# westlake-repl/Adapter4Rec

Measured on NVIDIA B200. Metric: train user-sequences/s (SASRec + BERT-base LoRA r=8 adapter-tuning step: fwd+bwd+allreduce+Adam), higher is better.
Workload: dtype bf16

## Files before the change

adapter4rec_b200/csrc/attention_small.cu:

```cuda
#include "a4r_common.cuh"
#include "mma_sync.cuh"

namespace {

constexpr int LP = 32;
constexpr int WARPS_PER_CTA = 4;

struct AttnParams {
  const __nv_bfloat16* qkv;
  __nv_bfloat16* out;
  const __nv_bfloat16* dout;
  const void* mask;
  int64_t ld_qkv, ld_out, mask_ld;
  int N, L, heads;
  int mask_dtype;
  const int32_t* cu_seqlens;
  int causal;
  float scale, mask_neg;
  uint32_t drop_thr16;
  float drop_scale;
  uint64_t drop_seed, drop_offset;
};

A4R_DEVICE void prob_dropout(float (&s)[2][4][4], const AttnParams& p, int n, int h, int lane) {
// ... 237 lines not shown
      uint32_t a0[4], a1[4];
      acc_to_a(a0, s[0][2 * ks], s[0][2 * ks + 1]);
      acc_to_a(a1, s[1][2 * ks], s[1][2 * ks + 1]);
#pragma unroll
      for (int np = 0; np < DH / 16; ++np) {
        uint32_t b[4];
        load_b_kn<DH>(b, sV, np * 16, ks * 16, lane);
        const uint32_t b0[2] = {b[0], b[1]}, b1[2] = {b[2], b[3]};
        mma_bf16_16816(o[0][np * 2], a0, b0);
        mma_bf16_16816(o[0][np * 2 + 1], a0, b1);
        mma_bf16_16816(o[1][np * 2], a1, b0);
        mma_bf16_16816(o[1][np * 2 + 1], a1, b1);
      }
    }
    __syncwarp();
    acc_to_tile<DH, DH / 8>(my, o, 1.f, 1.f, 1.f, 1.f, lane);
    __syncwarp();
    store_tile<DH>(my, p.out + sq.row0 * p.ld_out + h * DH, p.ld_out, sq.L, lane);
    __syncwarp();
  }
}

template <int DH>
__global__ void __launch_bounds__(WARPS_PER_CTA * 32) attn_bwd_kernel(const AttnParams p) {
  extern __shared__ __align__(128) uint8_t smem_attn[];
  constexpr int TB = Tile<DH>::kBytes;
  constexpr int PB = Tile<32>::kBytes;
  const int warp = threadIdx.x >> 5, lane = threadIdx.x & 31;
  uint8_t* my = smem_attn + warp * (4 * TB + 2 * PB);
  const int64_t total = static_cast<int64_t>(p.N) * p.heads;
  for (int64_t w = static_cast<int64_t>(blockIdx.x) * WARPS_PER_CTA + warp; w < total;
       w += static_cast<int64_t>(gridDim.x) * WARPS_PER_CTA) {
    const int n = static_cast<int>(w / p.heads), h = static_cast<int>(w % p.heads);
    const int64_t Hd = static_cast<int64_t>(p.heads) * DH;
    const SeqSpan sq = seq_span(p, n);
    const __nv_bfloat16* q = p.qkv + sq.row0 * p.ld_qkv + h * DH;
    uint8_t *tQ = my, *tK = my + TB, *tV = my + 2 * TB, *tdO = my + 3 * TB, *tP = my + 4 * TB, *tdS = tP + PB;
    load_tile<DH>(tQ, q, p.ld_qkv, sq.L, lane);
    load_tile<DH>(tK, q + Hd, p.ld_qkv, sq.L, lane);
    load_tile<DH>(tV, q + 2 * Hd, p.ld_qkv, sq.L, lane);
    load_tile<DH>(tdO, p.dout + sq.row0 * p.ld_out + h * DH, p.ld_out, sq.L, lane);
    const uint32_t km = build_keymask(p, sq, lane);
    cp_async_wait_all();
    __syncwarp();
    const uint32_t sQ = smem_u32(tQ), sK = smem_u32(tK), sV = smem_u32(tV), sdO = smem_u32(tdO), sP = smem_u32(tP),
                   sdS = smem_u32(tdS);
    float s[2][4][4];
    scores_softmax<DH>(s, sQ, sK, p, sq.L, lane, km);
    float dp[2][4][4];
#pragma unroll
    for (int mt = 0; mt < 2; ++mt)
#pragma unroll
      for (int nt = 0; nt < 4; ++nt)
#pragma unroll
        for (int e = 0; e < 4; ++e) dp[mt][nt][e] = 0.0f;
#pragma unroll
// ... 94 lines not shown
        mma_bf16_16816(dk[0][np * 2 + 1], a0, b1);
        mma_bf16_16816(dk[1][np * 2], a1, b0);
        mma_bf16_16816(dk[1][np * 2 + 1], a1, b1);
        uint32_t c[4];
        load_b_kn<DH>(c, sdO, np * 16, ks * 16, lane);
        const uint32_t c0[2] = {c[0], c[1]}, c1[2] = {c[2], c[3]};
        mma_bf16_16816(dv[0][np * 2], p0, c0);
        mma_bf16_16816(dv[0][np * 2 + 1], p0, c1);
        mma_bf16_16816(dv[1][np * 2], p1, c0);
        mma_bf16_16816(dv[1][np * 2 + 1], p1, c1);
      }
    }
    __syncwarp();
    acc_to_tile<DH, DH / 8>(tQ, acc, 1.f, 1.f, 1.f, 1.f, lane);
    acc_to_tile<DH, DH / 8>(tK, dk, 1.f, 1.f, 1.f, 1.f, lane);
    acc_to_tile<DH, DH / 8>(tV, dv, 1.f, 1.f, 1.f, 1.f, lane);
    __syncwarp();
    __nv_bfloat16* dq = p.out + sq.row0 * p.ld_qkv + h * DH;
    store_tile<DH>(tQ, dq, p.ld_qkv, sq.L, lane);
    store_tile<DH>(tK, dq + Hd, p.ld_qkv, sq.L, lane);
    store_tile<DH>(tV, dq + 2 * Hd, p.ld_qkv, sq.L, lane);
    __syncwarp();
  }
}

int check_common(const a4r_attn_args* a) {
  A4R_CHECK_ARG(a != nullptr, "attention: args is NULL");
  A4R_CHECK_ARG(a->qkv && a->out, "attention: qkv/out must be non-NULL");
  A4R_CHECK_ARG(a->L >= 1 && a->L <= LP, "attention_small: L must be in [1,32] (got %lld)", (long long)a->L);
  A4R_CHECK_ARG(a->head_dim == 32 || a->head_dim == 64, "attention_small: head_dim must be 32 or 64");
  A4R_CHECK_ARG(a->heads >= 1 && a->N >= 0, "attention: bad heads/N");
  A4R_CHECK_ARG(a->ld_qkv >= 3 * a->heads * a->head_dim && a->ld_qkv % 8 == 0, "attention: bad ld_qkv");
  A4R_CHECK_ARG(a->ld_out >= a->heads * a->head_dim && a->ld_out % 8 == 0, "attention: bad ld_out");
  A4R_CHECK_ARG(a4r_aligned16(a->qkv) && a4r_aligned16(a->out), "attention: pointers must be 16B aligned");
  A4R_CHECK_ARG(a->mask_dtype >= 0 && a->mask_dtype <= 2, "attention: mask_dtype must be 0,1,2");
  if (a->mask_dtype != 0)
    A4R_CHECK_ARG(a->mask != nullptr && (a->cu_seqlens != nullptr || a->mask_ld >= a->L), "attention: bad mask/mask_ld");
  A4R_CHECK_ARG(a->dropout_p >= 0.0f && a->dropout_p < 1.0f, "attention: dropout_p must be in [0,1)");
  return a4r_device_check();
}

AttnParams to_params(const a4r_attn_args* a) {
  AttnParams p;
  p.qkv = static_cast<const __nv_bfloat16*>(a->qkv);
  p.out = static_cast<__nv_bfloat16*>(a->out);
  p.dout = static_cast<const __nv_bfloat16*>(a->dout);
// ... 38 lines not shown
  int rc = check_common(a);
  if (rc != A4R_OK) return rc;
  if (a->N == 0) return A4R_OK;
  const AttnParams p = to_params(a);
  static bool done64 = false, done32 = false;
  if (a->head_dim == 64)
    return launch(attn_fwd_kernel<64>, WARPS_PER_CTA * 3 * Tile<64>::kBytes, p, static_cast<cudaStream_t>(stream), &done64);
  return launch(attn_fwd_kernel<32>, WARPS_PER_CTA * 3 * Tile<32>::kBytes, p, static_cast<cudaStream_t>(stream), &done32);
}

extern "C" int a4r_attn_small_bwd(const a4r_attn_args* a, a4r_stream_t stream) {
  int rc = check_common(a);
  if (rc != A4R_OK) return rc;
  A4R_CHECK_ARG(a->dout != nullptr && a4r_aligned16(a->dout), "attention bwd: dout missing or unaligned");
  if (a->N == 0) return A4R_OK;
  const AttnParams p = to_params(a);
  static bool done64 = false, done32 = false;
  if (a->head_dim == 64)
    return launch(attn_bwd_kernel<64>, WARPS_PER_CTA * (4 * Tile<64>::kBytes + 2 * Tile<32>::kBytes), p,
                  static_cast<cudaStream_t>(stream), &done64);
  return launch(attn_bwd_kernel<32>, WARPS_PER_CTA * (4 * Tile<32>::kBytes + 2 * Tile<32>::kBytes), p,
                static_cast<cudaStream_t>(stream), &done32);
}
```

adapter4rec_b200/functional.py:

```python
import torch

from . import ops

BF16 = torch.bfloat16


PARAM_EPOCH = [0]


def bump_param_epoch():
    PARAM_EPOCH[0] += 1


class WeightCache:

    def __init__(self):
        self.key = None
        self.master = None
        self.w = None
        self.wt = None

    def get(self, weight, need_t=False):
        key = (weight.data_ptr(), weight._version, weight.device, PARAM_EPOCH[0] if weight.requires_grad else -1)
        if key != self.key:
# ... 256 lines not shown


def dropout_add(x, res, p):
    return DropoutAddFunction.apply(x, res, float(p))


class AddFunction(torch.autograd.Function):

    @staticmethod
    def forward(ctx, x, res):
        return ops.dropout(x.contiguous(), res.contiguous(), 0.0, 0, 0)

    @staticmethod
    def backward(ctx, dy):
        return (dy if ctx.needs_input_grad[0] else None), (dy if ctx.needs_input_grad[1] else None)


def add(x, res):
    return AddFunction.apply(x, res)


class AttentionFunction(torch.autograd.Function):
    @staticmethod
    def forward(ctx, qkv, mask, N, L, heads, head_dim, causal, mask_neg, dropout_p=0.0, scale=None, cu_seqlens=None):
        ctx.cfg = (N, L, heads, head_dim, causal, mask_neg, scale)
        ctx.cu = cu_seqlens
        ctx.mask = mask
        ctx.drop = None
        if dropout_p > 0.0:
            ctx.drop = (dropout_p,) + DropoutState.draw(N * heads * 32 * 8)
        out, lse = ops.attn_small_fwd(qkv, N, L, heads, head_dim, mask=mask, causal=causal, mask_neg=mask_neg, want_lse=True,
                                      dropout=ctx.drop, scale=scale, cu_seqlens=cu_seqlens)
        ctx.save_for_backward(qkv, lse, out if lse is not None else None)
        return out

    @staticmethod
    def backward(ctx, dctx):
        qkv, lse, out = ctx.saved_tensors
        N, L, heads, head_dim, causal, mask_neg, scale = ctx.cfg
        dqkv = ops.attn_small_bwd(qkv, dctx.contiguous(), N, L, heads, head_dim, mask=ctx.mask, causal=causal,
                                  mask_neg=mask_neg, lse=lse, ctx=out, dropout=ctx.drop, scale=scale, cu_seqlens=ctx.cu)
        return dqkv, None, None, None, None, None, None, None, None, None, None


def attention(qkv, mask, N, L, heads, head_dim, causal=False, mask_neg=ops.F32_MIN, dropout_p=0.0, scale=None,
              cu_seqlens=None):
    return AttentionFunction.apply(qkv, mask, N, L, heads, head_dim, causal, mask_neg, float(dropout_p), scale, cu_seqlens)


class GatherRowsFunction(torch.autograd.Function):

    @staticmethod
    def forward(ctx, x, idx):
        ctx.rows = x.shape[0]
        ctx.save_for_backward(idx)
        return ops.gather_rows(x.contiguous(), idx)

    @staticmethod
    def backward(ctx, dy):
        (idx,) = ctx.saved_tensors
        dx = torch.zeros((ctx.rows, dy.shape[1]), dtype=dy.dtype, device=dy.device)
        dx.index_copy_(0, idx, dy.contiguous())
        return dx, None


def gather_rows(x, idx):
    return GatherRowsFunction.apply(x, idx)


class ExpandRowsFunction(torch.autograd.Function):
# ... 94 lines not shown
                for j, o, r in slots:
                    st[0][o:o + r].copy_(params[4 * j + 2].detach())
                    torch.mul(params[4 * j + 3].detach(), 1.0 / r, out=st[1][j * H:(j + 1) * H, o:o + r])
                a_cat, a_cat_t = ops.cast_transpose(st[0], True, True)
                b_ext, b_ext_t = ops.cast_transpose(st[1], True, True)
                tb = cache.get("t_bias_const")
                if tb is None or tb[0] != ctx.ones_col or tb[1].device != dev:
                    t_bias = torch.zeros(LORA_PAD, dtype=torch.float32, device=dev)
                    if ctx.ones_col:
                        t_bias[LORA_PAD - 1] = 1.0
                    tb = cache["t_bias_const"] = (ctx.ones_col, t_bias)
                t_bias = tb[1]
                cache["a_cat"], cache["b_ext"], cache["t_bias"] = a_cat, b_ext, t_bias
                cache["a_cat_t"], cache["b_ext_t"] = a_cat_t, b_ext_t
            T = ops.gemm(x, a_cat, bias=t_bias)
            qkv = ops.gemm(x, w, bias=bias, a2=T, b2=b_ext)
        else:
            qkv = ops.gemm(x, w, bias=bias)
        ctx.cache, ctx.slots, ctx.H, ctx.n = cache, slots, H, n
        if not slots:
            ctx.ones_col = False
        ctx.n_params = len(params)
        ctx.param_needs = [p is not None and p.requires_grad for p in params]
        need_x = any(ctx.param_needs[4 * j + 2] for j in range(n)) or any(ctx.param_needs[4 * j] for j in range(n))
        ctx.save_for_backward(x if need_x else None, T, a_cat, b_ext)
        if ctx.with_skip:
            return qkv, x
        return qkv

    @staticmethod
    def backward(ctx, dqkv, dskip=None):
        x, T, a_cat, b_ext = ctx.saved_tensors
        H, cache, n = ctx.H, ctx.cache, ctx.n
        tail = (None,) if ctx.with_skip else ()
        if dqkv is None:
            return (dskip, None) + (None,) * ctx.n_params + tail
        dqkv = dqkv.contiguous()
        if dskip is not None:
            dskip = dskip.contiguous()
        if cache.get("wt") is None:
            cache["wt"] = cache["w"].t().contiguous()
        grads = [None] * ctx.n_params
        dT = None
        if ctx.slots:
            if cache.get("b_ext") is b_ext and cache.get("b_ext_t") is not None:
                b_ext_t, a_cat_t = cache["b_ext_t"], cache["a_cat_t"]
            else:
                b_ext_t, a_cat_t = b_ext.t().contiguous(), a_cat.t().contiguous()
                if cache.get("b_ext") is b_ext:
                    cache["b_ext_t"], cache["a_cat_t"] = b_ext_t, a_cat_t
            lj = [j for j, _, _ in ctx.slots]
            if n == 3 and len(lj) == 2:
                (ja, jb) = lj
                dT = ops.gemm(dqkv[:, ja * H:(ja + 1) * H], b_ext_t[:, ja * H:(ja + 1) * H],
                              a2=dqkv[:, jb * H:(jb + 1) * H], b2=b_ext_t[:, jb * H:(jb + 1) * H])
            elif n == 3 and len(lj) == 1:
                dT = ops.gemm(dqkv[:, lj[0] * H:(lj[0] + 1) * H], b_ext_t[:, lj[0] * H:(lj[0] + 1) * H])
            else:
                dT = ops.gemm(dqkv, b_ext_t)
            dx = ops.gemm(dqkv, cache["wt"], a2=dT, b2=a_cat_t, residual=dskip) if ctx.needs_input_grad[0] else None
        else:
            dx = ops.gemm(dqkv, cache["wt"], residual=dskip) if ctx.needs_input_grad[0] else None
        fused = bool(ctx.slots) and ctx.ones_col
        if fused:
            want_g1 = any(ctx.param_needs[4 * j + 1] for j in range(n)) or any(ctx.param_needs[4 * j + 3] for j, _, _ in ctx.slots)
            want_g2 = any(ctx.param_needs[4 * j + 2] for j, _, _ in ctx.slots)
            g1_rows = [ctx.param_needs[4 * j + 1] or any(jj == j and ctx.param_needs[4 * j + 3] for jj, _, _ in ctx.slots)
                       for j in range(n)]
            g1 = [None] * n
            if want_g1:
                if all(g1_rows):
                    full = ops.wgrad(dqkv, T)
                    g1 = [full[j * H:(j + 1) * H] for j in range(n)]
                else:
                    g1 = [ops.wgrad(dqkv[:, j * H:(j + 1) * H], T) if g1_rows[j] else None for j in range(n)]
            g2 = ops.wgrad(dT, x) if want_g2 else None
        for j in range(n):
            dq = dqkv[:, j * H:(j + 1) * H]
            if ctx.param_needs[4 * j]:
                grads[4 * j] = ops.wgrad(dq, x)
            if ctx.param_needs[4 * j + 1]:
                grads[4 * j + 1] = g1[j][:, LORA_PAD - 1].contiguous() if fused else ops.colsum(dq)
        for j, o, r in ctx.slots:
            dq = dqkv[:, j * H:(j + 1) * H]
            if ctx.param_needs[4 * j + 3]:
                grads[4 * j + 3] = (g1[j][:, o:o + r] * (1.0 / r)) if fused else \
                    _pad_cols_wgrad(dq, T, o, r, 1.0 / r, transpose=False)
            if ctx.param_needs[4 * j + 2]:
                grads[4 * j + 2] = g2[o:o + r].contiguous() if fused else _pad_cols_wgrad(dT, x, o, r, 1.0, transpose=True)
        return (dx, None) + tuple(grads) + tail


def _pad_cols_wgrad(a, b, off, r, alpha, transpose):
    lo = (off // 8) * 8
    hi = ((off + r + 7) // 8) * 8
    if transpose:
        full = ops.wgrad(a[:, lo:hi], b, alpha=alpha)
        return full[off - lo:off - lo + r].contiguous()
    full = ops.wgrad(a, b[:, lo:hi], alpha=alpha)
    return full[:, off - lo:off - lo + r].contiguous()


class EmbedLNFunction(torch.autograd.Function):

    @staticmethod
    def forward(ctx, ids, L, tables, gamma, beta, eps, roberta_pad_id, prompt, word_pad_idx, *params):
        word, pos, typ = tables
        need_prompt = prompt is not None and prompt.requires_grad
        need_tab = [p is not None and p.requires_grad for p in params] + [False] * (5 - len(params))
        need = need_prompt or any(need_tab)
# ... 254 lines not shown
```

adapter4rec_b200/lib.py:

```python
import ctypes
import os
from ctypes import POINTER, Structure, c_char_p, c_float, c_int32, c_int64, c_size_t, c_void_p

HERE = os.path.dirname(os.path.abspath(__file__))
LIB_PATH = os.path.join(HERE, "libadapter4rec_sm100.so")

A4R_OK, A4R_EINVAL, A4R_ECUDA, A4R_EARCH, A4R_EWORKSPACE = 0, -1, -2, -3, -4
EPI_LINEAR, EPI_GELU, EPI_RELU, EPI_DGELU, EPI_DRELU = 0, 1, 2, 3, 4


class GemmArgs(Structure):
    _fields_ = [
        ("A", c_void_p), ("lda", c_int64), ("B", c_void_p), ("ldb", c_int64),
        ("A2", c_void_p), ("lda2", c_int64), ("B2", c_void_p), ("ldb2", c_int64), ("K2", c_int64),
        ("C", c_void_p), ("ldc", c_int64), ("aux", c_void_p), ("ldaux", c_int64),
        ("residual", c_void_p), ("ldr", c_int64), ("residual2", c_void_p), ("ldr2", c_int64),
        ("bias", c_void_p), ("M", c_int64), ("N", c_int64), ("K", c_int64),
        ("alpha", c_float), ("epilogue", c_int32), ("out_f32", c_int32), ("block_n", c_int32),
        ("dropout_p", c_float), ("dropout_seed", ctypes.c_uint64), ("dropout_offset", ctypes.c_uint64),
        ("dropout_after_residual", c_int32),
    ]


class AttnArgs(Structure):
    _fields_ = [
        ("qkv", c_void_p), ("out", c_void_p), ("dout", c_void_p), ("mask", c_void_p),
        ("ld_qkv", c_int64), ("ld_out", c_int64), ("mask_ld", c_int64),
        ("N", c_int64), ("L", c_int64), ("heads", c_int64), ("head_dim", c_int64),
        ("mask_dtype", c_int32), ("causal", c_int32), ("scale", c_float), ("mask_neg", c_float),
        ("lse", c_void_p), ("ctx", c_void_p),
        ("dropout_p", c_float), ("dropout_seed", ctypes.c_uint64), ("dropout_offset", ctypes.c_uint64),
        ("cu_seqlens", c_void_p),
    ]


class EmbedArgs(Structure):
    _fields_ = [
        ("ids", c_void_p), ("ld_ids", c_int64), ("word_emb", c_void_p), ("pos_emb", c_void_p),
        ("type_emb", c_void_p), ("prompt", c_void_p), ("gamma", c_void_p), ("beta", c_void_p),
        ("out", c_void_p), ("z_out", c_void_p), ("mean_out", c_void_p), ("rstd_out", c_void_p),
        ("N", c_int64), ("L", c_int64), ("H", c_int64), ("pos_offset", c_int64),
        ("roberta_pad_id", c_int64), ("n_prompt", c_int64), ("eps", c_float),
    ]


class BceArgs(Structure):
    _fields_ = [
        ("prec", c_void_p), ("emb", c_void_p), ("log_mask", c_void_p), ("pos_score", c_void_p),
        ("neg_score", c_void_p), ("loss", c_void_p), ("count", c_void_p),
        ("B", c_int64), ("S", c_int64), ("D", c_int64), ("cpc", c_int32),
    ]


class AdapterArgs(Structure):
    _fields_ = [
# ... 2 lines not shown
        ("gamma", c_void_p), ("beta", c_void_p), ("out", c_void_p), ("z_out", c_void_p),
        ("mean", c_void_p), ("rstd", c_void_p), ("s_out", c_void_p), ("u_out", c_void_p),
        ("M", c_int64), ("H", c_int64), ("r", c_int64), ("act", c_int32), ("tail", c_int32), ("eps", c_float),
        ("lds", c_int64), ("impl", c_int32),
    ]


class InbatchCeArgs(Structure):
    _fields_ = [
        ("prec", c_void_p), ("cand", c_void_p), ("ld_cand", c_int64), ("item_ids", c_void_p), ("log_mask", c_void_p),
        ("cand_bias", c_void_p), ("lse", c_void_p), ("loss", c_void_p), ("count", c_void_p),
        ("B", c_int64), ("S", c_int64), ("D", c_int64), ("masked_logit", c_float),
    ]


PROTOTYPES = {
    "a4r_version": (c_int32, []),
    "a4r_last_error_string": (c_char_p, []),
    "a4r_device_check": (c_int32, []),
    "a4r_launch_count": (c_int64, []),
    "a4r_gemm_bf16_tn": (c_int32, [POINTER(GemmArgs), c_void_p]),
    "a4r_attn_small_fwd": (c_int32, [POINTER(AttnArgs), c_void_p]),
    "a4r_attn_small_bwd": (c_int32, [POINTER(AttnArgs), c_void_p]),
    "a4r_attn_mid_fwd": (c_int32, [POINTER(AttnArgs), c_void_p]),
    "a4r_attn_mid_bwd": (c_int32, [POINTER(AttnArgs), c_void_p]),
    "a4r_layernorm_fwd": (c_int32, [c_void_p, c_void_p, c_int64, c_void_p, c_void_p, c_float, c_void_p, c_void_p,
                                    c_void_p, c_void_p, c_int64, c_int64, c_void_p]),
    "a4r_layernorm_bwd_workspace_bytes": (c_size_t, [c_int64]),
    "a4r_layernorm_bwd": (c_int32, [c_void_p, c_void_p, c_void_p, c_void_p, c_void_p, c_void_p, c_void_p, c_void_p,
                                    c_int32, c_void_p, c_size_t, c_int64, c_int64, c_void_p, c_float, ctypes.c_uint64,
                                    ctypes.c_uint64, c_void_p]),
    "a4r_layernorm_bwd_add": (c_int32, [c_void_p, c_void_p, c_void_p, c_void_p, c_void_p, c_void_p, c_void_p, c_int64, c_int64,
                                        c_void_p]),
    "a4r_adapter_ln_supported": (c_int32, [c_int64, c_int64]),
    "a4r_adapter_ln_fwd": (c_int32, [POINTER(AdapterArgs), c_void_p]),
    "a4r_embed_ln_fwd": (c_int32, [POINTER(EmbedArgs), c_void_p]),
    "a4r_act_bwd": (c_int32, [c_void_p, c_void_p, c_void_p, c_int64, c_int32, c_void_p]),
    "a4r_act_fwd": (c_int32, [c_void_p, c_void_p, c_int64, c_int32, c_void_p]),
    "a4r_scatter_add_rows": (c_int32, [c_void_p, c_int64, c_void_p, c_void_p, c_int64, c_int64, c_int64, c_int64, c_void_p]),
    "a4r_cast_transpose_f32_bf16": (c_int32, [c_void_p, c_int64, c_void_p, c_void_p, c_int64, c_int64, c_void_p]),
    "a4r_dropout": (c_int32, [c_void_p, c_void_p, c_void_p, c_int64, c_float, ctypes.c_uint64, ctypes.c_uint64, c_void_p]),
    "a4r_colsum_workspace_bytes": (c_size_t, [c_int64]),
    "a4r_colsum": (c_int32, [c_void_p, c_int64, c_int64, c_int64, c_void_p, c_int32, c_void_p, c_size_t, c_void_p]),
    "a4r_wgrad_workspace_bytes": (c_size_t, [c_int64, c_int64, c_int64]),
    "a4r_wgrad_bf16": (c_int32, [c_void_p, c_int64, c_void_p, c_int64, c_void_p, c_int64, c_int64, c_int64, c_int64,
                                 c_float, c_int32, c_void_p, c_size_t, c_void_p]),
# ... 57 lines not shown
```

adapter4rec_b200/model/bert.py:

```python
import torch
import torch.nn as nn

from .. import functional as Fn
from .. import ops
from .layers import BF16, Embedding, LayerNorm, Linear, LoRALinear, to_2d_bf16


class TextConfigLite:

    def __init__(self, hf_config=None, **kw):
        src = {} if hf_config is None else {k: getattr(hf_config, k) for k in dir(hf_config) if not k.startswith("_")
                                            and isinstance(getattr(hf_config, k, None), (int, float, str, bool, type(None)))}
        src.update(kw)
        self.vocab_size = src.get("vocab_size", 30522)
        self.hidden_size = src.get("hidden_size", 768)
        self.num_hidden_layers = src.get("num_hidden_layers", 12)
        self.num_attention_heads = src.get("num_attention_heads", 12)
        self.intermediate_size = src.get("intermediate_size", 3072)
        self.max_position_embeddings = src.get("max_position_embeddings", 512)
        self.type_vocab_size = src.get("type_vocab_size", 2)
        self.layer_norm_eps = src.get("layer_norm_eps", 1e-12)
        self.pad_token_id = src.get("pad_token_id", 0)
        self.model_type = src.get("model_type", "bert")
        self.hidden_dropout_prob = src.get("hidden_dropout_prob", 0.1)
# ... 26 lines not shown
        tables = (table, self.position_embeddings.table_bf16(), typ)
        g, b = self.LayerNorm.weight.detach().float(), self.LayerNorm.bias.detach().float()
        wmaster = we.wte.weight if hasattr(we, "learned_embedding") else we.weight
        masters = [wmaster, self.position_embeddings.weight, self.token_type_embeddings.weight, self.LayerNorm.weight,
                   self.LayerNorm.bias]
        masters = [m if m.requires_grad else None for m in masters]
        x = Fn.EmbedLNFunction.apply(input_ids, L, tables, g, b, self.LayerNorm.eps, roberta_pad, prompt,
                                     int(self.config.pad_token_id), *masters)
        if self.training and self.dropout.p > 0:
            x = Fn.dropout_add(x, None, self.dropout.p)
        return x


class BertSelfAttention(nn.Module):
    def __init__(self, config):
        super().__init__()
        self.num_attention_heads = config.num_attention_heads
        self.attention_head_size = config.hidden_size // config.num_attention_heads
        self.all_head_size = config.hidden_size
        self.query = Linear(config.hidden_size, config.hidden_size)
        self.key = Linear(config.hidden_size, config.hidden_size)
        self.value = Linear(config.hidden_size, config.hidden_size)
        self.dropout = nn.Dropout(config.attention_probs_dropout_prob)
        self._qkv_cache = {}

    def forward(self, x2d, attention_mask, N, L, packed=None, want_skip=False):
        params = []
        for m in (self.query, self.key, self.value):
            params += [m.weight, m.bias, getattr(m, "lora_A", None), getattr(m, "lora_B", None)]
        skip = x2d
        if want_skip and x2d.requires_grad:
            qkv, skip = Fn.QKVFunction.apply(x2d, self._qkv_cache, *params, "skip")
        else:
            qkv = Fn.QKVFunction.apply(x2d, self._qkv_cache, *params)
        if packed is not None:
            ctx = Fn.attention(qkv, packed.token_mask, N, L, self.num_attention_heads, self.attention_head_size,
                               causal=False, mask_neg=ops.F32_MIN, dropout_p=self.dropout.p if self.training else 0.0,
                               cu_seqlens=packed.cu_seqlens)
        else:
            ctx = Fn.attention(qkv, attention_mask, N, L, self.num_attention_heads, self.attention_head_size,
                               causal=False, mask_neg=ops.F32_MIN, dropout_p=self.dropout.p if self.training else 0.0)
        return (ctx, skip) if want_skip else ctx


class BertSelfOutput(nn.Module):

    def __init__(self, config, in_features=None):
        super().__init__()
        self.dense = Linear(in_features or config.hidden_size, config.hidden_size)
        self.LayerNorm = LayerNorm(config.hidden_size, eps=config.layer_norm_eps)
        self.dropout = nn.Dropout(config.hidden_dropout_prob)

    def forward(self, hidden_states, input_tensor):
        shape = input_tensor.shape
        p = self.dropout.p if self.training else 0.0
        d = self.dense
        if not (d.weight.requires_grad or d.bias.requires_grad):
            out = Fn.PostLNBlockFunction.apply(to_2d_bf16(hidden_states), to_2d_bf16(input_tensor), self.LayerNorm.weight,
                                               self.LayerNorm.bias, self.LayerNorm.eps, p, d.weight, d.bias, d._cache,
                                               None, None, None)
            return out.view(shape)
        if p > 0:
            z = Fn.dropout_add(d(to_2d_bf16(hidden_states)), to_2d_bf16(input_tensor).contiguous(), p)
        else:
# ... 150 lines not shown
```

adapter4rec_b200/ops.py:

```python
import ctypes

import torch

from . import lib as _l
from .lib import EPI_DGELU, EPI_DRELU, EPI_GELU, EPI_LINEAR, EPI_RELU

BF16 = torch.bfloat16
F32_MIN = -3.4028234663852886e38


def _stream():
    return ctypes.c_void_p(torch.cuda.current_stream().cuda_stream)


def _p(t):
    return None if t is None else ctypes.c_void_p(t.data_ptr())


def _rows2d(t, name):
    if t.dim() != 2 or t.stride(1) != 1:
        raise ValueError("%s must be 2-D with unit column stride, got shape %s stride %s" % (name, tuple(t.shape), t.stride()))
    return t.stride(0) if t.shape[0] > 1 else max(t.stride(0), t.shape[1])


# ... 132 lines not shown
        lse = torch.empty((N * L, heads), dtype=torch.float32, device=qkv.device)
        a.lse = _p(lse)
    fn, name = _attn_kernel(L, head_dim, causal, "fwd")
    _l.check(fn(ctypes.byref(a), _stream()), name)
    return (out, lse) if want_lse else out


def attn_small_bwd(qkv, dctx, N, L, heads, head_dim, mask=None, causal=False, mask_neg=F32_MIN, lse=None, ctx=None,
                   dropout=None, scale=None, cu_seqlens=None):
    assert qkv.dtype == BF16 and dctx.dtype == BF16 and dctx.shape[0] == qkv.shape[0]
    assert cu_seqlens is not None or qkv.shape[0] == N * L
    dqkv = torch.empty((qkv.shape[0], 3 * heads * head_dim), dtype=BF16, device=qkv.device)
    a = _attn_args(qkv, N, L, heads, head_dim, mask, causal, mask_neg, dropout, scale, cu_seqlens)
    assert _rows2d(qkv, "qkv") == dqkv.stride(0), "attention bwd expects a contiguous qkv"
    a.out, a.dout, a.ld_out = _p(dqkv), _p(dctx), _rows2d(dctx, "dctx")
    if L > 32:
        assert lse is not None and ctx is not None and ctx.is_contiguous() and dctx.is_contiguous()
        a.lse, a.ctx = _p(lse), _p(ctx)
    fn, name = _attn_kernel(L, head_dim, causal, "bwd")
    _l.check(fn(ctypes.byref(a), _stream()), name)
    return dqkv


def layernorm_fwd(x, gamma, beta, eps, res=None, want_z=False, want_stats=True):
    assert x.dtype == BF16 and x.is_contiguous() and x.dim() == 2
    M, H = x.shape
    y = torch.empty_like(x)
    z = torch.empty_like(x) if want_z else None
    mean = torch.empty(M, dtype=torch.float32, device=x.device) if want_stats else None
    rstd = torch.empty(M, dtype=torch.float32, device=x.device) if want_stats else None
    res_rows = 0
    if res is not None:
        assert res.dtype == BF16 and res.is_contiguous() and res.shape[-1] == H
        res_rows = res.numel() // H
    _l.check(_l.get_lib().a4r_layernorm_fwd(_p(x), _p(res), res_rows, _p(gamma), _p(beta), float(eps), _p(y), _p(z),
                                            _p(mean), _p(rstd), M, H, _stream()), "a4r_layernorm_fwd")
    return y, z, mean, rstd


def layernorm_bwd(dy, z, mean, rstd, gamma, dgamma=None, dbeta=None, accumulate=False, masked=None):
    assert dy.dtype == BF16 and z.dtype == BF16 and dy.is_contiguous() and z.is_contiguous()
    M, H = z.shape
    dz = torch.empty_like(z)
    dzm = torch.empty_like(z) if masked is not None else None
    mp, mseed, moff = masked if masked is not None else (0.0, 0, 0)
    ws, wsb = None, 0
# ... 389 lines not shown
```

include/adapter4rec.h:

```cpp
#ifndef ADAPTER4REC_H_
#define ADAPTER4REC_H_

#include <stddef.h>
#include <stdint.h>

#ifdef __cplusplus
extern "C" {
#endif

#define A4R_OK 0
#define A4R_EINVAL (-1)
#define A4R_ECUDA (-2)
#define A4R_EARCH (-3)
#define A4R_EWORKSPACE (-4)

typedef void* a4r_stream_t;

#define A4R_API __attribute__((visibility("default")))

A4R_API int a4r_version(void);
A4R_API const char* a4r_last_error_string(void);
A4R_API int a4r_device_check(void);
A4R_API int64_t a4r_launch_count(void);

// ... 39 lines not shown

typedef struct a4r_attn_args {
  const void* qkv;
  void* out;
  const void* dout;
  const void* mask;
  int64_t ld_qkv, ld_out, mask_ld;
  int64_t N, L, heads, head_dim;
  int32_t mask_dtype;
  int32_t causal;
  float scale;
  float mask_neg;
  float* lse;
  const void* ctx;
  float dropout_p;
  uint64_t dropout_seed;
  uint64_t dropout_offset;
  const int32_t* cu_seqlens;
} a4r_attn_args;

A4R_API int a4r_attn_small_fwd(const a4r_attn_args* args, a4r_stream_t stream);
A4R_API int a4r_attn_small_bwd(const a4r_attn_args* args, a4r_stream_t stream);

A4R_API int a4r_attn_mid_fwd(const a4r_attn_args* args, a4r_stream_t stream);
A4R_API int a4r_attn_mid_bwd(const a4r_attn_args* args, a4r_stream_t stream);

A4R_API int a4r_layernorm_fwd(const void* x, const void* res, int64_t res_rows, const float* gamma, const float* beta,
                      float eps, void* y, void* z_out, float* mean, float* rstd, int64_t M, int64_t H,
                      a4r_stream_t stream);
A4R_API size_t a4r_layernorm_bwd_workspace_bytes(int64_t H);
A4R_API int a4r_layernorm_bwd(const void* dy, const void* z, const float* mean, const float* rstd, const float* gamma,
                      void* dz, float* dgamma, float* dbeta, int32_t accumulate, void* workspace,
                      size_t workspace_bytes, int64_t M, int64_t H, void* dz_masked, float dropout_p,
                      uint64_t dropout_seed, uint64_t dropout_offset, a4r_stream_t stream);
A4R_API int a4r_layernorm_bwd_add(const void* dy, const void* z, const float* mean, const float* rstd, const float* gamma,
                          const void* dskip, void* dz, int64_t M, int64_t H, a4r_stream_t stream);

typedef struct a4r_adapter_args {
  const void* h;
  int64_t ldh;
  const void* input;
  int64_t ldi;
  const void* w_down;
  const float* b_down;
  const void* w_up;
  const float* b_up;
// ... 136 lines not shown
```

Baseline: 2010.

## Fuse LoRA-B gradient and dT computation into the attention backward kernel via clusters

New measurement: 1733, median of 6. -13.8%, worse.

```diff
diff --git a/adapter4rec_b200/csrc/attention_small.cu b/adapter4rec_b200/csrc/attention_small.cu
--- a/adapter4rec_b200/csrc/attention_small.cu
+++ b/adapter4rec_b200/csrc/attention_small.cu
@@ -283,16 +283,10 @@
 }
 
 template <int DH>
-__global__ void __launch_bounds__(WARPS_PER_CTA * 32) attn_bwd_kernel(const AttnParams p) {
-  extern __shared__ __align__(128) uint8_t smem_attn[];
+A4R_DEVICE void bwd_head(const AttnParams& p, int n, int h, uint8_t* my, int lane) {
   constexpr int TB = Tile<DH>::kBytes;
   constexpr int PB = Tile<32>::kBytes;
-  const int warp = threadIdx.x >> 5, lane = threadIdx.x & 31;
-  uint8_t* my = smem_attn + warp * (4 * TB + 2 * PB);
-  const int64_t total = static_cast<int64_t>(p.N) * p.heads;
-  for (int64_t w = static_cast<int64_t>(blockIdx.x) * WARPS_PER_CTA + warp; w < total;
-       w += static_cast<int64_t>(gridDim.x) * WARPS_PER_CTA) {
-    const int n = static_cast<int>(w / p.heads), h = static_cast<int>(w % p.heads);
+  {
     const int64_t Hd = static_cast<int64_t>(p.heads) * DH;
     const SeqSpan sq = seq_span(p, n);
     const __nv_bfloat16* q = p.qkv + sq.row0 * p.ld_qkv + h * DH;
@@ -433,6 +427,194 @@
     store_tile<DH>(tV, dq + 2 * Hd, p.ld_qkv, sq.L, lane);
     __syncwarp();
   }
+}
+
+template <int DH>
+__global__ void __launch_bounds__(WARPS_PER_CTA * 32) attn_bwd_kernel(const AttnParams p) {
+  extern __shared__ __align__(128) uint8_t smem_attn[];
+  const int warp = threadIdx.x >> 5, lane = threadIdx.x & 31;
+  uint8_t* my = smem_attn + warp * (4 * Tile<DH>::kBytes + 2 * Tile<32>::kBytes);
+  const int64_t total = static_cast<int64_t>(p.N) * p.heads;
+  for (int64_t w = static_cast<int64_t>(blockIdx.x) * WARPS_PER_CTA + warp; w < total;
+       w += static_cast<int64_t>(gridDim.x) * WARPS_PER_CTA)
+    bwd_head<DH>(p, static_cast<int>(w / p.heads), static_cast<int>(w % p.heads), my, lane);
+}
+
+constexpr int LORA_W = 8;
+constexpr int LORA_G = LORA_W + 1;
+constexpr int kLoraStage = 32 * 2 * LORA_W;
+constexpr int kLoraAcc = 2 * 64 * LORA_G;
+constexpr int kLoraTiles = 4 * Tile<64>::kBytes + 2 * Tile<32>::kBytes;
+constexpr int kLoraSmem = WARPS_PER_CTA * (kLoraTiles + 4 * (kLoraStage + kLoraAcc));
+
+struct LoraParams {
+  const __nv_bfloat16* t;
+  const __nv_bfloat16* b_ext_t;
+  __nv_bfloat16* dt;
+  float* partial;
+  int64_t ld_t, ld_b, ld_dt;
+  int off[2], rank[2];
+};
+
+A4R_DEVICE void cluster_arrive() { asm volatile("barrier.cluster.arrive.release.aligned;" ::: "memory"); }
+A4R_DEVICE void cluster_wait() { asm volatile("barrier.cluster.wait.acquire.aligned;" ::: "memory"); }
+A4R_DEVICE float ld_cluster_f32(uint32_t addr) {
+  float v;
+  asm volatile("ld.shared::cluster.f32 %0, [%1];" : "=f"(v) : "r"(addr) : "memory");
+  return v;
+}
+A4R_DEVICE uint32_t ld_bf16_bits(const __nv_bfloat16* p) {
+  return static_cast<uint32_t>(__bfloat16_as_ushort(__ldg(p)));
+}
+
+__global__ void __launch_bounds__(WARPS_PER_CTA * 32) attn_bwd_lora_kernel(const AttnParams p, const LoraParams lp) {
+  extern __shared__ __align__(128) uint8_t smem_attn[];
+  constexpr int TB = Tile<64>::kBytes;
+  const int warp = threadIdx.x >> 5, lane = threadIdx.x & 31, g = lane >> 2, t = lane & 3;
+  uint8_t* my = smem_attn + warp * kLoraTiles;
+  float* stage = reinterpret_cast<float*>(smem_attn + WARPS_PER_CTA * kLoraTiles);
+  float* gacc = stage + WARPS_PER_CTA * kLoraStage + warp * kLoraAcc;
+  uint32_t cid, ncl;
+  asm("mov.u32 %0, %%clusterid.x;" : "=r"(cid));
+  asm("mov.u32 %0, %%nclusterid.x;" : "=r"(ncl));
+  const int csize = p.heads / WARPS_PER_CTA;
+  const int h = static_cast<int>(cluster_ctarank()) * WARPS_PER_CTA + warp;
+  const int64_t H = static_cast<int64_t>(p.heads) * 64;
+  for (int i = lane; i < kLoraAcc; i += 32) gacc[i] = 0.0f;
+  bool first = true;
+  for (int n = static_cast<int>(cid); n < p.N; n += static_cast<int>(ncl)) {
+    bwd_head<64>(p, n, h, my, lane);
+    const SeqSpan sq = seq_span(p, n);
+    const uint32_t tile[2] = {smem_u32(my), smem_u32(my + 2 * TB)};
+    float dt[2][2][4];
+#pragma unroll
+    for (int s = 0; s < 2; ++s) {
+#pragma unroll
+      for (int e = 0; e < 4; ++e) dt[0][s][e] = dt[1][s][e] = 0.0f;
+      const bool ok = g < lp.rank[s];
+      const __nv_bfloat16* bsrc = lp.b_ext_t + static_cast<int64_t>(lp.off[s] + (ok ? g : 0)) * lp.ld_b + s * 2 * H + h * 64 + 2 * t;
+#pragma unroll
+      for (int ks = 0; ks < 4; ++ks) {
+        const uint32_t b[2] = {ok ? __ldg(reinterpret_cast<const uint32_t*>(bsrc + ks * 16)) : 0u,
+                               ok ? __ldg(reinterpret_cast<const uint32_t*>(bsrc + ks * 16 + 8)) : 0u};
+        uint32_t a0[4], a1[4];
+        load_a<64>(a0, tile[s], 0, ks * 16, lane);
+        load_a<64>(a1, tile[s], 16, ks * 16, lane);
+        mma_bf16_16816(dt[0][s], a0, b);
+        mma_bf16_16816(dt[1][s], a1, b);
+      }
+    }
+    const __nv_bfloat16* trow = lp.t + sq.row0 * lp.ld_t;
+    uint32_t tb[3][2][2];
+#pragma unroll
+    for (int ks = 0; ks < 2; ++ks)
+#pragma unroll
+      for (int hf = 0; hf < 2; ++hf) {
+        const int i0 = ks * 16 + hf * 8 + 2 * t;
+#pragma unroll
+        for (int s = 0; s < 3; ++s) {
+          const bool ok = s < 2 ? g < lp.rank[s] : g == 0;
+          const int c = s < 2 ? lp.off[s] + g : 63;
+          const uint32_t lo = ok && i0 < sq.L ? ld_bf16_bits(trow + static_cast<int64_t>(i0) * lp.ld_t + c) : 0u;
+          const uint32_t hi = ok && i0 + 1 < sq.L ? ld_bf16_bits(trow + static_cast<int64_t>(i0 + 1) * lp.ld_t + c) : 0u;
+          tb[s][ks][hf] = lo | (hi << 16);
+        }
+      }
+#pragma unroll
+    for (int s = 0; s < 2; ++s) {
+      float gw[4][2][4];
+#pragma unroll
+      for (int mt = 0; mt < 4; ++mt)
+#pragma unroll
+        for (int e = 0; e < 4; ++e) gw[mt][0][e] = gw[mt][1][e] = 0.0f;
+#pragma unroll
+      for (int ks = 0; ks < 2; ++ks)
+#pragma unroll
+        for (int mt = 0; mt < 4; ++mt) {
+          uint32_t a[4];
+          load_a_t<64>(a, tile[s], mt * 16, ks * 16, lane);
+          mma_bf16_16816(gw[mt][0], a, tb[s][ks]);
+          mma_bf16_16816(gw[mt][1], a, tb[2][ks]);
+        }
+      float* G = gacc + s * 64 * LORA_G;
+#pragma unroll
+      for (int mt = 0; mt < 4; ++mt) {
+        const int d0 = mt * 16 + g;
+        G[d0 * LORA_G + 2 * t] += gw[mt][0][0];
+        G[d0 * LORA_G + 2 * t + 1] += gw[mt][0][1];
+        G[(d0 + 8) * LORA_G + 2 * t] += gw[mt][0][2];
+        G[(d0 + 8) * LORA_G + 2 * t + 1] += gw[mt][0][3];
+        if (t == 0) {
+          G[d0 * LORA_G + LORA_W] += gw[mt][1][0];
+          G[(d0 + 8) * LORA_G + LORA_W] += gw[mt][1][2];
+        }
+      }
+    }
+    if (!first) cluster_wait();
+    first = false;
+    float* st = stage + warp * kLoraStage;
+#pragma unroll
+    for (int mt = 0; mt < 2; ++mt)
+#pragma unroll
+      for (int s = 0; s < 2; ++s) {
+        const int r0 = mt * 16 + g, c = s * LORA_W + 2 * t;
+        st[r0 * 16 + c] = dt[mt][s][0];
+        st[r0 * 16 + c + 1] = dt[mt][s][1];
+        st[(r0 + 8) * 16 + c] = dt[mt][s][2];
+        st[(r0 + 8) * 16 + c + 1] = dt[mt][s][3];
+      }
+    cluster_arrive();
+    cluster_wait();
+    const uint32_t st0 = smem_u32(stage);
+    for (int pr = static_cast<int>(cluster_ctarank()) * 128 + threadIdx.x; pr < sq.L * 32; pr += csize * 128) {
+      const int row = pr >> 5, c0 = (pr & 31) * 2;
+      float v[2];
+#pragma unroll
+      for (int e = 0; e < 2; ++e) {
+        const int c = c0 + e;
+        int idx = -1;
+        if (c >= lp.off[0] && c < lp.off[0] + lp.rank[0]) idx = c - lp.off[0];
+        else if (c >= lp.off[1] && c < lp.off[1] + lp.rank[1]) idx = LORA_W + c - lp.off[1];
+        float acc = 0.0f;
+        if (idx >= 0)
+          for (int hh = 0; hh < p.heads; ++hh)
+            acc += ld_cluster_f32(mapa_u32(st0 + 4u * ((hh % WARPS_PER_CTA) * kLoraStage + row * 16 + idx), hh / WARPS_PER_CTA));
+        v[e] = acc;
+      }
+      *reinterpret_cast<uint32_t*>(lp.dt + (sq.row0 + row) * lp.ld_dt + c0) = pack_bf16x2(v[0], v[1]);
+    }
+    cluster_arrive();
+  }
+  if (!first) cluster_wait();
+  __syncwarp();
+  float* out = lp.partial + static_cast<int64_t>(cid) * 2 * H * LORA_G;
+  for (int i = lane; i < kLoraAcc; i += 32) {
+    const int s = i / (64 * LORA_G), rem = i % (64 * LORA_G);
+    out[s * H * LORA_G + h * 64 * LORA_G + rem] = gacc[i];
+  }
+}
+
+struct LoraOut {
+  float* grad_b[2];
+  float* grad_bias[2];
+  int rank[2];
+  float inv_rank[2];
+};
+
+__global__ void lora_grad_reduce_kernel(const float* __restrict__ partial, int ncl, int cols, const LoraOut o) {
+  const int i = blockIdx.x * blockDim.x + threadIdx.x;
+  const int per = cols * LORA_G;
+  if (i >= 2 * per) return;
+  float acc = 0.0f;
+  for (int c = 0; c < ncl; ++c) acc += partial[static_cast<int64_t>(c) * 2 * per + i];
+  const int s = i / per, col = (i % per) / LORA_G, k = i % LORA_G;
+  if (k < o.rank[s]) o.grad_b[s][col * o.rank[s] + k] = acc * o.inv_rank[s];
+  else if (k == LORA_W && o.grad_bias[s] != nullptr) o.grad_bias[s][col] = acc;
+}
+
+int lora_clusters(int64_t N, int64_t heads) {
+  const int64_t per = static_cast<int64_t>(a4r_num_sms()) * 2 / (heads / WARPS_PER_CTA);
+  return static_cast<int>(N < per ? N : per);
 }
 
 int check_common(const a4r_attn_args* a) {
@@ -517,3 +699,77 @@
   return launch(attn_bwd_kernel<32>, WARPS_PER_CTA * (4 * Tile<32>::kBytes + 2 * Tile<32>::kBytes), p,
                 static_cast<cudaStream_t>(stream), &done32);
 }
+
+extern "C" size_t a4r_attn_small_bwd_lora_workspace_bytes(int64_t N, int64_t heads) {
+  if (N <= 0 || heads < WARPS_PER_CTA || heads % WARPS_PER_CTA != 0) return 0;
+  return static_cast<size_t>(lora_clusters(N, heads)) * 2 * heads * 64 * LORA_G * sizeof(float);
+}
+
+extern "C" int a4r_attn_small_bwd_lora(const a4r_attn_lora_args* a, a4r_stream_t stream) {
+  A4R_CHECK_ARG(a != nullptr, "attention bwd lora: args is NULL");
+  const a4r_attn_args* at = &a->attn;
+  A4R_CHECK_ARG(at->head_dim == 64, "attention bwd lora: head_dim must be 64");
+  A4R_CHECK_ARG(at->heads >= WARPS_PER_CTA && at->heads % WARPS_PER_CTA == 0 && at->heads <= 8 * WARPS_PER_CTA,
+                "attention bwd lora: heads must be a multiple of 4 in [4, 32] (got %lld)", (long long)at->heads);
+  A4R_CHECK_ARG(a->t && a->b_ext_t && a->dt && a->grad_lora_b_q && a->grad_lora_b_v, "attention bwd lora: NULL operand");
+  A4R_CHECK_ARG(a4r_aligned16(a->t) && a4r_aligned16(a->b_ext_t) && a4r_aligned16(a->dt),
+                "attention bwd lora: T, B_ext_t and dT must be 16B aligned");
+  A4R_CHECK_ARG(a->ld_t >= 64 && a->ld_dt >= 64 && a->ld_dt % 2 == 0 && a->ld_b >= 3 * at->heads * 64 && a->ld_b % 2 == 0,
+                "attention bwd lora: bad leading dimensions");
+  A4R_CHECK_ARG(a->q_rank >= 1 && a->q_rank <= LORA_W && a->v_rank >= 1 && a->v_rank <= LORA_W,
+                "attention bwd lora: ranks must be in [1, 8]");
+  A4R_CHECK_ARG(a->q_off >= 0 && a->v_off >= 0 && a->q_off + a->q_rank <= 63 && a->v_off + a->v_rank <= 63 &&
+                    (a->q_off + a->q_rank <= a->v_off || a->v_off + a->v_rank <= a->q_off),
+                "attention bwd lora: slots must be disjoint and below column 63");
+  int rc = check_common(at);
+  if (rc != A4R_OK) return rc;
+  A4R_CHECK_ARG(at->dout != nullptr && a4r_aligned16(at->dout), "attention bwd: dout missing or unaligned");
+  const size_t need = a4r_attn_small_bwd_lora_workspace_bytes(at->N, at->heads);
+  if (a->workspace_bytes < need)
+    return a4r_set_error(A4R_EWORKSPACE, "attention bwd lora: workspace too small (%zu < %zu)", a->workspace_bytes, need);
+  A4R_CHECK_ARG(need == 0 || a4r_aligned16(a->workspace), "attention bwd lora: workspace must be 16B aligned");
+  const cudaStream_t st = static_cast<cudaStream_t>(stream);
+  const AttnParams p = to_params(at);
+  LoraParams lp;
+  lp.t = static_cast<const __nv_bfloat16*>(a->t);
+  lp.b_ext_t = static_cast<const __nv_bfloat16*>(a->b_ext_t);
+  lp.dt = static_cast<__nv_bfloat16*>(a->dt);
+  lp.partial = static_cast<float*>(a->workspace);
+  lp.ld_t = a->ld_t, lp.ld_b = a->ld_b, lp.ld_dt = a->ld_dt;
+  lp.off[0] = static_cast<int>(a->q_off), lp.off[1] = static_cast<int>(a->v_off);
+  lp.rank[0] = static_cast<int>(a->q_rank), lp.rank[1] = static_cast<int>(a->v_rank);
+  const int csize = static_cast<int>(at->heads / WARPS_PER_CTA);
+  const int ncl = at->N > 0 ? lora_clusters(at->N, at->heads) : 0;
+  if (ncl > 0) {
+    static bool done = false;
+    if (!done) {
+      A4R_CUDA_OK(cudaFuncSetAttribute(attn_bwd_lora_kernel, cudaFuncAttributeMaxDynamicSharedMemorySize, kLoraSmem));
+      done = true;
+    }
+    cudaLaunchConfig_t cfg = {};
+    cfg.gridDim = dim3(static_cast<unsigned>(ncl * csize));
+    cfg.blockDim = dim3(WARPS_PER_CTA * 32);
+    cfg.dynamicSmemBytes = kLoraSmem;
+    cfg.stream = st;
+    cudaLaunchAttribute attr[1];
+    attr[0].id = cudaLaunchAttributeClusterDimension;
+    attr[0].val.clusterDim.x = csize;
+    attr[0].val.clusterDim.y = 1;
+    attr[0].val.clusterDim.z = 1;
+    cfg.attrs = attr;
+    cfg.numAttrs = 1;
+    A4R_CUDA_OK(cudaLaunchKernelEx(&cfg, attn_bwd_lora_kernel, p, lp));
+    A4R_LAUNCH_OK();
+    a4r_count_launch(1);
+  }
+  LoraOut o;
+  o.grad_b[0] = a->grad_lora_b_q, o.grad_b[1] = a->grad_lora_b_v;
+  o.grad_bias[0] = a->grad_bias_q, o.grad_bias[1] = a->grad_bias_v;
+  o.rank[0] = lp.rank[0], o.rank[1] = lp.rank[1];
+  o.inv_rank[0] = 1.0f / static_cast<float>(lp.rank[0]), o.inv_rank[1] = 1.0f / static_cast<float>(lp.rank[1]);
+  const int cols = static_cast<int>(at->heads * 64);
+  lora_grad_reduce_kernel<<<(2 * cols * LORA_G + 255) / 256, 256, 0, st>>>(lp.partial, ncl, cols, o);
+  A4R_LAUNCH_OK();
+  a4r_count_launch(1);
+  return A4R_OK;
+}
diff --git a/adapter4rec_b200/functional.py b/adapter4rec_b200/functional.py
--- a/adapter4rec_b200/functional.py
+++ b/adapter4rec_b200/functional.py
@@ -1,3 +1,5 @@
+import os
+
 import torch
 
 from . import ops
@@ -302,10 +304,12 @@
 
 class AttentionFunction(torch.autograd.Function):
     @staticmethod
-    def forward(ctx, qkv, mask, N, L, heads, head_dim, causal, mask_neg, dropout_p=0.0, scale=None, cu_seqlens=None):
+    def forward(ctx, qkv, mask, N, L, heads, head_dim, causal, mask_neg, dropout_p=0.0, scale=None, cu_seqlens=None,
+                lora=None):
         ctx.cfg = (N, L, heads, head_dim, causal, mask_neg, scale)
         ctx.cu = cu_seqlens
         ctx.mask = mask
+        ctx.lora = lora
         ctx.drop = None
         if dropout_p > 0.0:
             ctx.drop = (dropout_p,) + DropoutState.draw(N * heads * 32 * 8)
@@ -318,14 +322,31 @@
     def backward(ctx, dctx):
         qkv, lse, out = ctx.saved_tensors
         N, L, heads, head_dim, causal, mask_neg, scale = ctx.cfg
-        dqkv = ops.attn_small_bwd(qkv, dctx.contiguous(), N, L, heads, head_dim, mask=ctx.mask, causal=causal,
-                                  mask_neg=mask_neg, lse=lse, ctx=out, dropout=ctx.drop, scale=scale, cu_seqlens=ctx.cu)
-        return dqkv, None, None, None, None, None, None, None, None, None, None
+        lora = ctx.lora
+        if lora is not None and head_dim == 64 and L <= 32 and heads % 4 == 0 and 4 <= heads <= 32:
+            dqkv, *lora.result = ops.attn_small_bwd_lora(
+                qkv, dctx.contiguous(), N, L, heads, ctx.mask, lora.T, lora.b_ext_t, lora.q_slot, lora.v_slot,
+                want_bias=lora.want_bias, causal=causal, mask_neg=mask_neg, dropout=ctx.drop, scale=scale, cu_seqlens=ctx.cu)
+        else:
+            dqkv = ops.attn_small_bwd(qkv, dctx.contiguous(), N, L, heads, head_dim, mask=ctx.mask, causal=causal,
+                                      mask_neg=mask_neg, lse=lse, ctx=out, dropout=ctx.drop, scale=scale, cu_seqlens=ctx.cu)
+        return dqkv, None, None, None, None, None, None, None, None, None, None, None
 
 
 def attention(qkv, mask, N, L, heads, head_dim, causal=False, mask_neg=ops.F32_MIN, dropout_p=0.0, scale=None,
-              cu_seqlens=None):
-    return AttentionFunction.apply(qkv, mask, N, L, heads, head_dim, causal, mask_neg, float(dropout_p), scale, cu_seqlens)
+              cu_seqlens=None, lora=None):
+    return AttentionFunction.apply(qkv, mask, N, L, heads, head_dim, causal, mask_neg, float(dropout_p), scale, cu_seqlens,
+                                   lora)
+
+
+LORA_ATTN_TAIL = os.environ.get("A4R_LORA_ATTN_TAIL", "1") != "0"
+
+
+class LoraTail:
+
+    def __init__(self, T, b_ext_t, q_slot, v_slot, want_bias):
+        self.T, self.b_ext_t, self.q_slot, self.v_slot, self.want_bias = T, b_ext_t, q_slot, v_slot, want_bias
+        self.result = None
 
 
 class GatherRowsFunction(torch.autograd.Function):
@@ -466,6 +487,12 @@
             ctx.ones_col = False
         ctx.n_params = len(params)
         ctx.param_needs = [p is not None and p.requires_grad for p in params]
+        ctx.tail = None
+        if (LORA_ATTN_TAIL and cache.get("lora_tail_wanted") and n == 3 and [j for j, _, _ in slots] == [0, 2] and ctx.ones_col
+                and all(r <= 8 for _, _, r in slots) and not ctx.param_needs[5]
+                and (ctx.param_needs[3] or ctx.param_needs[11])):
+            ctx.tail = LoraTail(T, cache["b_ext_t"], slots[0][1:], slots[1][1:], ctx.param_needs[1] or ctx.param_needs[9])
+            cache["lora_tail"] = ctx.tail
         need_x = any(ctx.param_needs[4 * j + 2] for j in range(n)) or any(ctx.param_needs[4 * j] for j in range(n))
         ctx.save_for_backward(x if need_x else None, T, a_cat, b_ext)
         if ctx.with_skip:
@@ -485,7 +512,10 @@
         if cache.get("wt") is None:
             cache["wt"] = cache["w"].t().contiguous()
         grads = [None] * ctx.n_params
-        dT = None
+        dT = lt = None
+        if ctx.tail is not None and ctx.tail.result is not None:
+            lt, ctx.tail.result = ctx.tail.result, None
+            dT = lt[0]
         if ctx.slots:
             if cache.get("b_ext") is b_ext and cache.get("b_ext_t") is not None:
                 b_ext_t, a_cat_t = cache["b_ext_t"], cache["a_cat_t"]
@@ -494,7 +524,9 @@
                 if cache.get("b_ext") is b_ext:
                     cache["b_ext_t"], cache["a_cat_t"] = b_ext_t, a_cat_t
             lj = [j for j, _, _ in ctx.slots]
-            if n == 3 and len(lj) == 2:
+            if lt is not None:
+                pass
+            elif n == 3 and len(lj) == 2:
                 (ja, jb) = lj
                 dT = ops.gemm(dqkv[:, ja * H:(ja + 1) * H], b_ext_t[:, ja * H:(ja + 1) * H],
                               a2=dqkv[:, jb * H:(jb + 1) * H], b2=b_ext_t[:, jb * H:(jb + 1) * H])
@@ -512,7 +544,7 @@
             g1_rows = [ctx.param_needs[4 * j + 1] or any(jj == j and ctx.param_needs[4 * j + 3] for jj, _, _ in ctx.slots)
                        for j in range(n)]
             g1 = [None] * n
-            if want_g1:
+            if want_g1 and lt is None:
                 if all(g1_rows):
                     full = ops.wgrad(dqkv, T)
                     g1 = [full[j * H:(j + 1) * H] for j in range(n)]
@@ -524,12 +556,18 @@
             if ctx.param_needs[4 * j]:
                 grads[4 * j] = ops.wgrad(dq, x)
             if ctx.param_needs[4 * j + 1]:
-                grads[4 * j + 1] = g1[j][:, LORA_PAD - 1].contiguous() if fused else ops.colsum(dq)
+                if lt is not None:
+                    grads[4 * j + 1] = lt[3 + j // 2]
+                else:
+                    grads[4 * j + 1] = g1[j][:, LORA_PAD - 1].contiguous() if fused else ops.colsum(dq)
         for j, o, r in ctx.slots:
             dq = dqkv[:, j * H:(j + 1) * H]
             if ctx.param_needs[4 * j + 3]:
-                grads[4 * j + 3] = (g1[j][:, o:o + r] * (1.0 / r)) if fused else \
-                    _pad_cols_wgrad(dq, T, o, r, 1.0 / r, transpose=False)
+                if lt is not None:
+                    grads[4 * j + 3] = lt[1 + j // 2]
+                else:
+                    grads[4 * j + 3] = (g1[j][:, o:o + r] * (1.0 / r)) if fused else \
+                        _pad_cols_wgrad(dq, T, o, r, 1.0 / r, transpose=False)
             if ctx.param_needs[4 * j + 2]:
                 grads[4 * j + 2] = g2[o:o + r].contiguous() if fused else _pad_cols_wgrad(dT, x, o, r, 1.0, transpose=True)
         return (dx, None) + tuple(grads) + tail
diff --git a/adapter4rec_b200/lib.py b/adapter4rec_b200/lib.py
--- a/adapter4rec_b200/lib.py
+++ b/adapter4rec_b200/lib.py
@@ -31,6 +31,15 @@
         ("lse", c_void_p), ("ctx", c_void_p),
         ("dropout_p", c_float), ("dropout_seed", ctypes.c_uint64), ("dropout_offset", ctypes.c_uint64),
         ("cu_seqlens", c_void_p),
+    ]
+
+
+class AttnLoraArgs(Structure):
+    _fields_ = [
+        ("attn", AttnArgs), ("t", c_void_p), ("ld_t", c_int64), ("b_ext_t", c_void_p), ("ld_b", c_int64),
+        ("q_off", c_int64), ("q_rank", c_int64), ("v_off", c_int64), ("v_rank", c_int64),
+        ("dt", c_void_p), ("ld_dt", c_int64), ("grad_lora_b_q", c_void_p), ("grad_lora_b_v", c_void_p),
+        ("grad_bias_q", c_void_p), ("grad_bias_v", c_void_p), ("workspace", c_void_p), ("workspace_bytes", c_size_t),
     ]
 
 
@@ -79,6 +88,8 @@
     "a4r_gemm_bf16_tn": (c_int32, [POINTER(GemmArgs), c_void_p]),
     "a4r_attn_small_fwd": (c_int32, [POINTER(AttnArgs), c_void_p]),
     "a4r_attn_small_bwd": (c_int32, [POINTER(AttnArgs), c_void_p]),
+    "a4r_attn_small_bwd_lora_workspace_bytes": (c_size_t, [c_int64, c_int64]),
+    "a4r_attn_small_bwd_lora": (c_int32, [POINTER(AttnLoraArgs), c_void_p]),
     "a4r_attn_mid_fwd": (c_int32, [POINTER(AttnArgs), c_void_p]),
     "a4r_attn_mid_bwd": (c_int32, [POINTER(AttnArgs), c_void_p]),
     "a4r_layernorm_fwd": (c_int32, [c_void_p, c_void_p, c_int64, c_void_p, c_void_p, c_float, c_void_p, c_void_p,
diff --git a/adapter4rec_b200/model/bert.py b/adapter4rec_b200/model/bert.py
--- a/adapter4rec_b200/model/bert.py
+++ b/adapter4rec_b200/model/bert.py
@@ -72,7 +72,7 @@
         self.key = Linear(config.hidden_size, config.hidden_size)
         self.value = Linear(config.hidden_size, config.hidden_size)
         self.dropout = nn.Dropout(config.attention_probs_dropout_prob)
-        self._qkv_cache = {}
+        self._qkv_cache = {"lora_tail_wanted": True}
 
     def forward(self, x2d, attention_mask, N, L, packed=None, want_skip=False):
         params = []
@@ -83,13 +83,15 @@
             qkv, skip = Fn.QKVFunction.apply(x2d, self._qkv_cache, *params, "skip")
         else:
             qkv = Fn.QKVFunction.apply(x2d, self._qkv_cache, *params)
+        lora = self._qkv_cache.pop("lora_tail", None)
         if packed is not None:
             ctx = Fn.attention(qkv, packed.token_mask, N, L, self.num_attention_heads, self.attention_head_size,
                                causal=False, mask_neg=ops.F32_MIN, dropout_p=self.dropout.p if self.training else 0.0,
-                               cu_seqlens=packed.cu_seqlens)
+                               cu_seqlens=packed.cu_seqlens, lora=lora)
         else:
             ctx = Fn.attention(qkv, attention_mask, N, L, self.num_attention_heads, self.attention_head_size,
-                               causal=False, mask_neg=ops.F32_MIN, dropout_p=self.dropout.p if self.training else 0.0)
+                               causal=False, mask_neg=ops.F32_MIN, dropout_p=self.dropout.p if self.training else 0.0,
+                               lora=lora)
         return (ctx, skip) if want_skip else ctx
 
 
diff --git a/adapter4rec_b200/ops.py b/adapter4rec_b200/ops.py
--- a/adapter4rec_b200/ops.py
+++ b/adapter4rec_b200/ops.py
@@ -178,6 +178,34 @@
     return dqkv
 
 
+def attn_small_bwd_lora(qkv, dctx, N, L, heads, mask, T, b_ext_t, q_slot, v_slot, want_bias=True, causal=False,
+                        mask_neg=F32_MIN, dropout=None, scale=None, cu_seqlens=None):
+    assert qkv.dtype == BF16 and dctx.dtype == BF16 and dctx.shape[0] == qkv.shape[0] and L <= 32
+    assert cu_seqlens is not None or qkv.shape[0] == N * L
+    assert T.dtype == BF16 and b_ext_t.dtype == BF16 and T.shape == (qkv.shape[0], 64)
+    rows, H, dev = qkv.shape[0], heads * 64, qkv.device
+    dqkv = torch.empty((rows, 3 * H), dtype=BF16, device=dev)
+    dT = torch.empty((rows, 64), dtype=BF16, device=dev)
+    gbq = torch.empty((H, q_slot[1]), dtype=torch.float32, device=dev)
+    gbv = torch.empty((H, v_slot[1]), dtype=torch.float32, device=dev)
+    gq = torch.empty(H, dtype=torch.float32, device=dev) if want_bias else None
+    gv = torch.empty(H, dtype=torch.float32, device=dev) if want_bias else None
+    a = _l.AttnLoraArgs()
+    a.attn = _attn_args(qkv, N, L, heads, 64, mask, causal, mask_neg, dropout, scale, cu_seqlens)
+    assert _rows2d(qkv, "qkv") == dqkv.stride(0), "attention bwd expects a contiguous qkv"
+    a.attn.out, a.attn.dout, a.attn.ld_out = _p(dqkv), _p(dctx), _rows2d(dctx, "dctx")
+    a.t, a.ld_t = _p(T), _rows2d(T, "T")
+    a.b_ext_t, a.ld_b = _p(b_ext_t), _rows2d(b_ext_t, "b_ext_t")
+    a.q_off, a.q_rank, a.v_off, a.v_rank = int(q_slot[0]), int(q_slot[1]), int(v_slot[0]), int(v_slot[1])
+    a.dt, a.ld_dt = _p(dT), dT.stride(0)
+    a.grad_lora_b_q, a.grad_lora_b_v, a.grad_bias_q, a.grad_bias_v = _p(gbq), _p(gbv), _p(gq), _p(gv)
+    wsb = _l.get_lib().a4r_attn_small_bwd_lora_workspace_bytes(N, heads)
+    ws = workspace(wsb, dev)
+    a.workspace, a.workspace_bytes = _p(ws), ws.numel()
+    _l.check(_l.get_lib().a4r_attn_small_bwd_lora(ctypes.byref(a), _stream()), "a4r_attn_small_bwd_lora")
+    return dqkv, dT, gbq, gbv, gq, gv
+
+
 def layernorm_fwd(x, gamma, beta, eps, res=None, want_z=False, want_stats=True):
     assert x.dtype == BF16 and x.is_contiguous() and x.dim() == 2
     M, H = x.shape
diff --git a/include/adapter4rec.h b/include/adapter4rec.h
--- a/include/adapter4rec.h
+++ b/include/adapter4rec.h
@@ -85,6 +85,26 @@
 A4R_API int a4r_attn_small_fwd(const a4r_attn_args* args, a4r_stream_t stream);
 A4R_API int a4r_attn_small_bwd(const a4r_attn_args* args, a4r_stream_t stream);
 
+typedef struct a4r_attn_lora_args {
+  a4r_attn_args attn;
+  const void* t;
+  int64_t ld_t;
+  const void* b_ext_t;
+  int64_t ld_b;
+  int64_t q_off, q_rank, v_off, v_rank;
+  void* dt;
+  int64_t ld_dt;
+  float* grad_lora_b_q;
+  float* grad_lora_b_v;
+  float* grad_bias_q;
+  float* grad_bias_v;
+  void* workspace;
+  size_t workspace_bytes;
+} a4r_attn_lora_args;
+
+A4R_API size_t a4r_attn_small_bwd_lora_workspace_bytes(int64_t N, int64_t heads);
+A4R_API int a4r_attn_small_bwd_lora(const a4r_attn_lora_args* args, a4r_stream_t stream);
+
 A4R_API int a4r_attn_mid_fwd(const a4r_attn_args* args, a4r_stream_t stream);
 A4R_API int a4r_attn_mid_bwd(const a4r_attn_args* args, a4r_stream_t stream);
 
```
